# lxa9867/ImageFolder

Measured on NVIDIA H100. Metric: tokenizer_train_images_per_sec_256x256, higher is better.
Workload: dtype bf16

## Files before the change

imagefolder_b200/csrc/attn_kernel.cu:

```cuda
#include "xq_common.cuh"
#include "xq_tc.cuh"

namespace xq {
using namespace xqtc;

constexpr int AT_BM = 128;
constexpr int AT_BN = 128;
constexpr int AT_D = 64;
constexpr int AT_NS = 2;
constexpr int AT_TILE = AT_BM * AT_D * 2;
constexpr int AT_THREADS = 288;

struct AttnFwdSmem {
    static constexpr int Q = 0;
    static constexpr int K = AT_TILE;
    static constexpr int V = AT_TILE * (1 + AT_NS);
    static constexpr int BAR = AT_TILE * (1 + 2 * AT_NS);
    static constexpr int BYTES = BAR + 256;
};

__device__ __forceinline__ void named_bar_sync(int id, int nthreads) { asm volatile("bar.sync %0, %1;" ::"r"(id), "r"(nthreads) : "memory"); }

__global__ void __launch_bounds__(AT_THREADS, 1)
attn_fwd_kernel(const __grid_constant__ CUtensorMap tmQKV, __nv_bfloat16 *__restrict__ out, float *__restrict__ lse2, int N, int H,
// ... 135 lines not shown
attn_fwd_tail_kernel(const __nv_bfloat16 *__restrict__ qkv, __nv_bfloat16 *__restrict__ out, float *__restrict__ lse2, int B, int N,
                     int H, int n0 , float c) {
    const int lane = threadIdx.x & 31;
    const long long w = ((long long)blockIdx.x * blockDim.x + threadIdx.x) >> 5;
    const int nt = N - n0;
    if (w >= (long long)B * H * nt) return;
    const int r = (int)(w % nt);
    const int bh = (int)(w / nt);
    const int b = bh / H, h = bh - b * H;
    const int n = n0 + r;
    const size_t W = (size_t)3 * H * AT_D;
    const __nv_bfloat16 *qp = qkv + ((size_t)b * N + n) * W + h * AT_D;
    float qf[AT_D];
#pragma unroll
    for (int u = 0; u < 8; ++u) {
        const uint4 x = *reinterpret_cast<const uint4 *>(qp + u * 8);
        const __nv_bfloat162 *x2 = reinterpret_cast<const __nv_bfloat162 *>(&x);
#pragma unroll
        for (int e = 0; e < 4; ++e) {
            const float2 f = __bfloat1622float2(x2[e]);
            qf[u * 8 + 2 * e] = f.x * c;
            qf[u * 8 + 2 * e + 1] = f.y * c;
        }
    }
    float m = -CUDART_INF_F, l = 0.f, o[AT_D];
#pragma unroll
    for (int i = 0; i < AT_D; ++i) o[i] = 0.f;
    for (int key = lane; key < N; key += 32) {
        const __nv_bfloat16 *kp = qkv + ((size_t)b * N + key) * W + (H + h) * AT_D;
        const __nv_bfloat16 *vp = kp + (size_t)H * AT_D;
        float s = 0.f;
#pragma unroll
        for (int u = 0; u < 8; ++u) {
            const uint4 x = *reinterpret_cast<const uint4 *>(kp + u * 8);
            const __nv_bfloat162 *x2 = reinterpret_cast<const __nv_bfloat162 *>(&x);
#pragma unroll
            for (int e = 0; e < 4; ++e) {
                const float2 f = __bfloat1622float2(x2[e]);
                s = fmaf(qf[u * 8 + 2 * e], f.x, s);
                s = fmaf(qf[u * 8 + 2 * e + 1], f.y, s);
            }
        }
        const float m_new = fmaxf(m, s);
        const float corr = ex2_approx(m - m_new);
        const float p = ex2_approx(s - m_new);
        l = fmaf(l, corr, p);
        m = m_new;
#pragma unroll
        for (int u = 0; u < 8; ++u) {
            const uint4 x = *reinterpret_cast<const uint4 *>(vp + u * 8);
            const __nv_bfloat162 *x2 = reinterpret_cast<const __nv_bfloat162 *>(&x);
#pragma unroll
            for (int e = 0; e < 4; ++e) {
                const float2 f = __bfloat1622float2(x2[e]);
                o[u * 8 + 2 * e] = fmaf(o[u * 8 + 2 * e], corr, p * f.x);
                o[u * 8 + 2 * e + 1] = fmaf(o[u * 8 + 2 * e + 1], corr, p * f.y);
            }
        }
    }
    float M = m;
#pragma unroll
    for (int off = 16; off > 0; off >>= 1) M = fmaxf(M, __shfl_xor_sync(0xffffffffu, M, off));
    const float f = (m == -CUDART_INF_F) ? 0.f : ex2_approx(m - M);
    l *= f;
#pragma unroll
    for (int off = 16; off > 0; off >>= 1) l += __shfl_xor_sync(0xffffffffu, l, off);
    const float inv = 1.0f / l;
    float mine0 = 0.f, mine1 = 0.f;
#pragma unroll
    for (int i = 0; i < AT_D; ++i) {
        float x = o[i] * f;
#pragma unroll
        for (int off = 16; off > 0; off >>= 1) x += __shfl_xor_sync(0xffffffffu, x, off);
        if (i == 2 * lane) mine0 = x;
        if (i == 2 * lane + 1) mine1 = x;
    }
    __nv_bfloat16 *op = out + ((size_t)b * N + n) * H * AT_D + h * AT_D;
    *reinterpret_cast<uint32_t *>(op + 2 * lane) = pack_bf16(mine0 * inv, mine1 * inv);
    if (lane == 0) lse2[(size_t)bh * N + n] = M + log2f(l);
}

constexpr int AB_THREADS = 288;
constexpr int AB_BQ = 64;
constexpr int AB_QS = 3;
constexpr int AB_QTILE = AB_BQ * AT_D * 2;

struct AttnBwdSmem {
    static constexpr int K = 0;
    static constexpr int V = AT_TILE;
    static constexpr int Q = 2 * AT_TILE;
    static constexpr int DO = Q + AB_QS * AB_QTILE;
    static constexpr int DS = DO + AB_QS * AB_QTILE;
    static constexpr int STAT = DS + 2 * AB_QTILE;
    static constexpr int BAR = STAT + AB_QS * 512;
    static constexpr int BYTES = BAR + 256;
};

__device__ __forceinline__ void bwd_epilogue_frag(const float (&acc)[32], float mul, __nv_bfloat16 *__restrict__ row0,
                                                  size_t row_stride, bool ok0, bool ok1, float *__restrict__ g_bias_cols, int lane) {
    const int cq = 2 * (lane & 3);
#pragma unroll
    for (int jj = 0; jj < AT_D / 8; ++jj) {
        const uint32_t w0 = pack_bf16(acc[4 * jj] * mul, acc[4 * jj + 1] * mul);
        const uint32_t w1 = pack_bf16(acc[4 * jj + 2] * mul, acc[4 * jj + 3] * mul);
        if (ok0) *reinterpret_cast<uint32_t *>(row0 + 8 * jj + cq) = w0;
        if (ok1) *reinterpret_cast<uint32_t *>(row0 + 8 * row_stride + 8 * jj + cq) = w1;
        if (g_bias_cols) {
            float s0 = __uint_as_float(w0 << 16) + __uint_as_float(w1 << 16);
            float s1 = __uint_as_float(w0 & 0xffff0000u) + __uint_as_float(w1 & 0xffff0000u);
#pragma unroll
            for (int o = 4; o < 32; o <<= 1) {
                s0 += __shfl_xor_sync(0xffffffffu, s0, o);
                s1 += __shfl_xor_sync(0xffffffffu, s1, o);
            }
            if (lane < 4) {
                atomicAdd(g_bias_cols + 8 * jj + cq, s0);
                atomicAdd(g_bias_cols + 8 * jj + cq + 1, s1);
            }
        }
    }
}

__global__ void __launch_bounds__(AB_THREADS, 1)
attn_bwd_kernel(const __grid_constant__ CUtensorMap tmQKV, const __grid_constant__ CUtensorMap tmDO, const float *__restrict__ lseP,
                const float *__restrict__ deltaP, float *__restrict__ dq_acc, __nv_bfloat16 *__restrict__ dqkv, float *__restrict__ g_bias,
                int N, int H, int Npad, float c, float scale) {
    extern __shared__ uint8_t smem_raw[];
    uint8_t *base = (uint8_t *)(((uintptr_t)smem_raw + 1023) & ~(uintptr_t)1023);
    uint64_t *bars = (uint64_t *)(base + AttnBwdSmem::BAR);
    uint64_t *kv_full = bars;
    uint64_t *q_full = bars + 1;
    uint64_t *q_empty = bars + 1 + AB_QS;
    float *s_lse = (float *)(base + AttnBwdSmem::STAT);
    float *s_delta = s_lse + AB_QS * AB_BQ;

    const int tid = threadIdx.x, warp = tid >> 5, lane = tid & 31;
    const int bh = blockIdx.y, b = bh / H, h = bh - b * H;
    const int k0 = blockIdx.x * AT_BN;
    const int colQ = h * AT_D, colK = (H + h) * AT_D, colV = (2 * H + h) * AT_D;
    const int nQ = (N + AB_BQ - 1) / AB_BQ;

    if (tid == 0) {
        mbar_init(kv_full, 1);
        for (int i = 0; i < AB_QS; ++i) { mbar_init(&q_full[i], 1); mbar_init(&q_empty[i], 8); }
        mbar_fence_init();
    }
    __syncthreads();

    if (warp == 8) {
        if (elect_one()) {
            tma_prefetch_desc(&tmQKV);
            tma_prefetch_desc(&tmDO);
            mbar_expect_tx(kv_full, 2 * AT_TILE);
            for (int hf = 0; hf < 2; ++hf) {
                tma_load_3d(base + AttnBwdSmem::K + hf * AB_QTILE, &tmQKV, colK, k0 + hf * AB_BQ, b, kv_full);
                tma_load_3d(base + AttnBwdSmem::V + hf * AB_QTILE, &tmQKV, colV, k0 + hf * AB_BQ, b, kv_full);
            }
        }
        __syncwarp();
        for (int i = 0; i < nQ; ++i) {
            const int st = i % AB_QS;
            mbar_wait(&q_empty[st], ((i / AB_QS) & 1) ^ 1);
            if (elect_one()) {
                mbar_expect_tx(&q_full[st], 2 * AB_QTILE + 2 * AB_BQ * 4);
                tma_load_3d(base + AttnBwdSmem::Q + st * AB_QTILE, &tmQKV, colQ, i * AB_BQ, b, &q_full[st]);
                tma_load_3d(base + AttnBwdSmem::DO + st * AB_QTILE, &tmDO, h * AT_D, i * AB_BQ, b, &q_full[st]);
                bulk_g2s(s_lse + st * AB_BQ, lseP + (size_t)bh * Npad + i * AB_BQ, AB_BQ * 4, &q_full[st]);
                bulk_g2s(s_delta + st * AB_BQ, deltaP + (size_t)bh * Npad + i * AB_BQ, AB_BQ * 4, &q_full[st]);
            }
            __syncwarp();
        }
        return;
    }

    const int wg = warp >> 2, wq = warp & 3;
    const int rq = wq * 16 + (lane >> 2), cq = 2 * (lane & 3);
    const int key0 = k0 + wg * 64 + rq;
    const bool kok0 = key0 < N, kok1 = key0 + 8 < N;
    const uint32_t kw = smem_u32(base + AttnBwdSmem::K + wg * AB_QTILE), vw = smem_u32(base + AttnBwdSmem::V + wg * AB_QTILE);
    const uint64_t kd_k = desc_k_sw128(kw), vd_k = desc_k_sw128(vw), kd_mn = desc_mn_sw128(kw, AT_TILE);
    const uint32_t dsw = smem_u32(base + AttnBwdSmem::DS + wg * AB_QTILE);
    const uint64_t dsd = desc_mn_sw128(dsw, AT_TILE);
    float dv[32], dk[32];
#pragma unroll
    for (int i = 0; i < 32; ++i) dv[i] = dk[i] = 0.f;
    mbar_wait(kv_full, 0);
    for (int i = 0; i < nQ; ++i) {
        const int st = i % AB_QS;
        mbar_wait(&q_full[st], (i / AB_QS) & 1);
        const uint32_t qa = smem_u32(base + AttnBwdSmem::Q + st * AB_QTILE), da = smem_u32(base + AttnBwdSmem::DO + st * AB_QTILE);
        float s[32], dp[32];
        wgmma_fence();
#pragma unroll
        for (int k = 0; k < AT_D / 16; ++k) wgmma_m64n64k16_ss<0, 0>(s, desc_adv(kd_k, k * 32), desc_adv(desc_k_sw128(qa), k * 32), (uint32_t)k);
#pragma unroll
        for (int k = 0; k < AT_D / 16; ++k) wgmma_m64n64k16_ss<0, 0>(dp, desc_adv(vd_k, k * 32), desc_adv(desc_k_sw128(da), k * 32), (uint32_t)k);
        wgmma_commit();
        wgmma_wait<0>();
        fence_regs(s);
        fence_regs(dp);
        const float *L = s_lse + st * AB_BQ, *D = s_delta + st * AB_BQ;
        uint32_t pa[4][4], sa[4][4];
#pragma unroll
        for (int jj = 0; jj < AB_BQ / 8; ++jj) {
            const float2 Lq = *reinterpret_cast<const float2 *>(L + 8 * jj + cq);
            const float2 Dq = *reinterpret_cast<const float2 *>(D + 8 * jj + cq);
#pragma unroll
            for (int hh = 0; hh < 2; ++hh) {
                const bool ok = hh ? kok1 : kok0;
                const float p0 = ok ? ex2_approx(fmaf(s[4 * jj + 2 * hh], c, -Lq.x)) : 0.f;
                const float p1 = ok ? ex2_approx(fmaf(s[4 * jj + 2 * hh + 1], c, -Lq.y)) : 0.f;
                const uint32_t pw = pack_bf16(p0, p1);
                const float d0 = __uint_as_float(pw << 16) * (dp[4 * jj + 2 * hh] - Dq.x);
                const float d1 = __uint_as_float(pw & 0xffff0000u) * (dp[4 * jj + 2 * hh + 1] - Dq.y);
                const uint32_t dw = pack_bf16(d0, d1);
                pa[jj >> 1][(jj & 1) * 2 + hh] = pw;
                sa[jj >> 1][(jj & 1) * 2 + hh] = dw;
                asm volatile("st.shared.b32 [%0], %1;" ::"r"(dsw + rowtile_off_bf16(rq + 8 * hh, 8 * jj + cq)), "r"(dw) : "memory");
            }
        }
        fence_async_smem();
        named_bar_sync(1 + wg, 128);
        const uint64_t qd_mn = desc_mn_sw128(qa, AT_TILE), dd_mn = desc_mn_sw128(da, AT_TILE);
        float dq[32];
        wgmma_fence();
#pragma unroll
        for (int k = 0; k < AB_BQ / 16; ++k) {
            wgmma_m64n64k16_rs<1>(dv, pa[k], desc_adv(dd_mn, k * 2048), 1u);
            wgmma_m64n64k16_rs<1>(dk, sa[k], desc_adv(qd_mn, k * 2048), 1u);
        }
#pragma unroll
        for (int k = 0; k < 64 / 16; ++k) wgmma_m64n64k16_ss<1, 1>(dq, desc_adv(dsd, k * 2048), desc_adv(kd_mn, k * 2048), (uint32_t)k);
        wgmma_commit();
        wgmma_wait<0>();
        fence_regs(dv);
        fence_regs(dk);
        fence_regs(dq);
        __syncwarp();
        if (lane == 0) mbar_arrive(&q_empty[st]);
        named_bar_sync(1 + wg, 128);
#pragma unroll
        for (int hh = 0; hh < 2; ++hh) {
            const int q = i * AB_BQ + rq + 8 * hh;
            if (q < N) {
                float *dst = dq_acc + ((size_t)bh * N + q) * AT_D + cq;
#pragma unroll
                for (int jj = 0; jj < AT_D / 8; ++jj)
                    atomicAdd(reinterpret_cast<float2 *>(dst + 8 * jj), make_float2(dq[4 * jj + 2 * hh], dq[4 * jj + 2 * hh + 1]));
            }
        }
    }
    const size_t W = (size_t)3 * H * AT_D;
    __nv_bfloat16 *row = dqkv + ((size_t)b * N + key0) * W;
    bwd_epilogue_frag(dv, 1.0f, row + colV, W, kok0, kok1, g_bias ? g_bias + colV : nullptr, lane);
    bwd_epilogue_frag(dk, scale, row + colK, W, kok0, kok1, g_bias ? g_bias + colK : nullptr, lane);
}


constexpr int AB_KTAIL_MAX = 4;
constexpr int AB_PREP_ROWS = 128;

__device__ __forceinline__ void unpack8(const uint4 &w, float (&f)[8]) {
    const uint32_t x[4] = {w.x, w.y, w.z, w.w};
#pragma unroll
    for (int e = 0; e < 4; ++e) { f[2 * e] = __uint_as_float(x[e] << 16); f[2 * e + 1] = __uint_as_float(x[e] & 0xffff0000u); }
}

template <int NT>
__global__ void __launch_bounds__(256, 2)
attn_bwd_prep_kernel(const __nv_bfloat16 *__restrict__ qkv, const __nv_bfloat16 *__restrict__ out, const __nv_bfloat16 *__restrict__ dout,
                     const float *__restrict__ lse2, float *__restrict__ lseP, float *__restrict__ deltaP, float *__restrict__ dq_acc,
                     float *__restrict__ dsT, __nv_bfloat16 *__restrict__ dqkv, float *__restrict__ g_bias, int N, int H, int Npad,
                     float c, float scale) {
    constexpr int NTA = NT > 0 ? NT : 1;
    __shared__ float red[NT > 0 ? 8 : 1][2][NTA][AT_D];
    __shared__ __align__(16) float skv[2][NTA][AT_D];
    const int bh = blockIdx.y, b = bh / H, h = bh - b * H;
    const int lane = threadIdx.x & 31, sub = threadIdx.x & 7, rloc = threadIdx.x >> 3;
    const int n0 = N - NT;
    const size_t W = (size_t)3 * H * AT_D;
    const __nv_bfloat16 *qb = qkv + (size_t)b * N * W + h * AT_D + sub * 8;
    const size_t ob = (size_t)b * N * H * AT_D + h * AT_D + sub * 8;
    float aK[NTA][8], aV[NTA][8];
    if constexpr (NT > 0) {
        if (threadIdx.x < NT * 16) {
            const int t = threadIdx.x >> 4, isv = (threadIdx.x >> 3) & 1;
            float f[8];
            unpack8(*reinterpret_cast<const uint4 *>(qb + (size_t)(n0 + t) * W + (size_t)(1 + isv) * H * AT_D), f);
#pragma unroll
            for (int e = 0; e < 8; ++e) skv[isv][t][sub * 8 + e] = f[e];
        }
#pragma unroll
        for (int t = 0; t < NT; ++t) {
#pragma unroll
            for (int e = 0; e < 8; ++e) aK[t][e] = aV[t][e] = 0.f;
        }
        __syncthreads();
    }
    constexpr int PASSES = AB_PREP_ROWS / 32;
    extern __shared__ uint4 prep_stage[];
    auto prefetch = [&](int blk, int stg) {
#pragma unroll
        for (int ps = 0; ps < PASSES; ++ps) {
            const int n = blk * AB_PREP_ROWS + ps * 32 + rloc;
            const int nc = n < N ? n : N - 1;
            uint4 *dst = prep_stage + ((size_t)(stg * 3) * PASSES + ps) * 256 + threadIdx.x;
            cp_async16(dst, out + ob + (size_t)nc * H * AT_D);
            cp_async16(dst + PASSES * 256, dout + ob + (size_t)nc * H * AT_D);
            cp_async16(dst + 2 * PASSES * 256, qb + (size_t)nc * W);
        }
        cp_async_commit();
    };
    if constexpr (NT > 0) prefetch(blockIdx.x, 0);
    int stg = 0;
    for (int blk = blockIdx.x; blk * AB_PREP_ROWS < Npad; blk += gridDim.x, stg ^= 1) {
        uint4 ow[PASSES], gw[PASSES], qw[PASSES];
        float lq[PASSES];
#pragma unroll
        for (int ps = 0; ps < PASSES; ++ps) {
            const int n = blk * AB_PREP_ROWS + ps * 32 + rloc;
            const int nc = n < N ? n : N - 1;
            if constexpr (NT == 0) {
                ow[ps] = *reinterpret_cast<const uint4 *>(out + ob + (size_t)nc * H * AT_D);
                gw[ps] = *reinterpret_cast<const uint4 *>(dout + ob + (size_t)nc * H * AT_D);
            }
            lq[ps] = lse2[(size_t)bh * N + nc];
        }
        if constexpr (NT > 0) {
            if ((blk + (int)gridDim.x) * AB_PREP_ROWS < Npad) { prefetch(blk + gridDim.x, stg ^ 1); cp_async_wait<1>(); }
            else cp_async_wait<0>();
        }
#pragma unroll
        for (int ps = 0; ps < PASSES; ++ps) {
            const int n = blk * AB_PREP_ROWS + ps * 32 + rloc;
// ... 130 lines not shown
        }
    }
    if (!g_bias) return;
#pragma unroll
    for (int e = 0; e < 8; ++e) {
        v[e] += __shfl_xor_sync(0xffffffffu, v[e], 8);
        v[e] += __shfl_xor_sync(0xffffffffu, v[e], 16);
    }
    const int warp = threadIdx.x >> 5, lane = threadIdx.x & 31;
    if (lane < 8) {
#pragma unroll
        for (int e = 0; e < 8; ++e) red[warp][lane * 8 + e] = v[e];
    }
    __syncthreads();
    if (threadIdx.x < AT_D) {
        float acc = 0.f;
#pragma unroll
        for (int w8 = 0; w8 < 8; ++w8) acc += red[w8][threadIdx.x];
        atomicAdd(g_bias + hh * AT_D + threadIdx.x, acc);
    }
}

static int attn_bwd_ktail(int N) {
    const int r = N % AT_BN;
    return (N > AT_BN && r != 0 && r <= AB_KTAIL_MAX) ? r : 0;
}

static size_t attn_bwd_ws_layout(int B, int N, int H, size_t *off_lse, size_t *off_delta, size_t *off_dst) {
    const size_t Npad = ((size_t)N + AT_BM - 1) / AT_BM * AT_BM;
    const size_t acc = align_up((size_t)B * H * N * AT_D * sizeof(float), 1024);
    const size_t st = align_up((size_t)B * H * Npad * sizeof(float), 1024);
    const size_t dst = align_up((size_t)B * H * N * attn_bwd_ktail(N) * sizeof(float), 1024);
    if (off_lse) *off_lse = acc;
    if (off_delta) *off_delta = acc + st;
    if (off_dst) *off_dst = acc + 2 * st;
    return acc + 2 * st + dst;
}

}

extern "C" {

size_t xq_vit_attn_bwd_workspace_bytes(int B, int N, int H) {
    if (B <= 0 || N <= 0 || H <= 0) return 0;
    return xq::attn_bwd_ws_layout(B, N, H, nullptr, nullptr, nullptr);
}

int xq_vit_attn_bwd(const void *qkv, const void *out, const void *d_out, const float *lse2, void *dqkv, float *g_bias, int B, int N,
                    int H, int head_dim, float scale, void *workspace, size_t workspace_bytes, void *stream) {
    using namespace xq;
    if (!qkv || !out || !d_out || !lse2 || !dqkv || !workspace || B <= 0 || N <= 0 || H <= 0) return XQ_ERR_ARG;
    if (head_dim != AT_D) return XQ_ERR_UNSUPPORTED;
    if (((uintptr_t)qkv & 15) || ((uintptr_t)out & 15) || ((uintptr_t)d_out & 15) || ((uintptr_t)dqkv & 15) || ((uintptr_t)workspace & 255))
        return XQ_ERR_ARG;
    size_t off_lse, off_delta, off_dst;
    if (workspace_bytes < attn_bwd_ws_layout(B, N, H, &off_lse, &off_delta, &off_dst)) return XQ_ERR_WORKSPACE;
    cudaStream_t st = (cudaStream_t)stream;
    float *acc = (float *)workspace;
    float *lseP = (float *)((char *)workspace + off_lse);
    float *deltaP = (float *)((char *)workspace + off_delta);
    float *dsT = (float *)((char *)workspace + off_dst);
    const uint64_t W = (uint64_t)3 * H * AT_D, Wo = (uint64_t)H * AT_D;
    CUtensorMap tmQKV, tmDO;
    if (!tensor_map_bf16_3d(&tmQKV, qkv, W, N, B, W * 2, (uint64_t)N * W * 2, AB_BQ) ||
        !tensor_map_bf16_3d(&tmDO, d_out, Wo, N, B, Wo * 2, (uint64_t)N * Wo * 2, AB_BQ))
        return XQ_ERR_UNSUPPORTED;
    const int nt = attn_bwd_ktail(N);
    const int nK = nt ? N / AT_BN : (N + AT_BN - 1) / AT_BN;
    const int Npad = (N + AT_BM - 1) / AT_BM * AT_BM;
    if ((long long)B * H > 65535) return XQ_ERR_UNSUPPORTED;
    if (g_bias) XQ_CUDA_TRY(cudaMemsetAsync(g_bias, 0, (size_t)3 * H * AT_D * sizeof(float), st));
    const float c2 = scale * 1.4426950408889634f;
    {
        dim3 grid(nt ? 1u : (unsigned)(Npad / AB_PREP_ROWS), (unsigned)(B * H));
        const size_t ps = nt ? (size_t)2 * 3 * (AB_PREP_ROWS / 32) * 256 * 16 : 0;
        decltype(&attn_bwd_prep_kernel<0>) const preps[] = {attn_bwd_prep_kernel<0>, attn_bwd_prep_kernel<1>, attn_bwd_prep_kernel<2>,
                                                            attn_bwd_prep_kernel<3>, attn_bwd_prep_kernel<4>};
        const auto prep = preps[nt < 4 ? nt : 4];
        if (int rc = smem_optin(prep, ps)) return rc;
        prep<<<grid, 256, ps, st>>>((const __nv_bfloat16 *)qkv, (const __nv_bfloat16 *)out, (const __nv_bfloat16 *)d_out, lse2, lseP,
                                    deltaP, acc, dsT, (__nv_bfloat16 *)dqkv, g_bias, N, H, Npad, c2, scale);
        XQ_LAUNCH_CHECK("attn_bwd_prep_kernel");
    }
    const size_t smem = AttnBwdSmem::BYTES + 1024;
    if (int rc = smem_optin(attn_bwd_kernel, smem)) return rc;
    attn_bwd_kernel<<<dim3((unsigned)nK, (unsigned)(B * H)), AB_THREADS, smem, st>>>(tmQKV, tmDO, lseP, deltaP, acc,
                                                                                     (__nv_bfloat16 *)dqkv, g_bias, N, H, Npad, c2, scale);
    XQ_LAUNCH_CHECK("attn_bwd_kernel");
    {
        dim3 grid((unsigned)((N + AB_CONV_ROWS - 1) / AB_CONV_ROWS), (unsigned)(B * H));
        attn_dq_convert_kernel<<<grid, 256, 0, st>>>(acc, (const __nv_bfloat16 *)qkv, dsT, (__nv_bfloat16 *)dqkv, g_bias, N, H, N - nt, nt, scale);
        XQ_LAUNCH_CHECK("attn_dq_convert_kernel");
    }
    return XQ_OK;
}

int xq_vit_attn_fwd(const void *qkv, void *out, float *lse2, int B, int N, int H, int head_dim, float scale, void *stream) {
    using namespace xq;
    if (!qkv || !out || !lse2 || B <= 0 || N <= 0 || H <= 0) return XQ_ERR_ARG;
    if (head_dim != AT_D) return XQ_ERR_UNSUPPORTED;
    if (((uintptr_t)qkv & 15) || ((uintptr_t)out & 15)) return XQ_ERR_ARG;
    const uint64_t W = (uint64_t)3 * H * AT_D;
    CUtensorMap tmQKV;
    if (!tensor_map_bf16_3d(&tmQKV, qkv, W, N, B, W * 2, (uint64_t)N * W * 2, AT_BM)) return XQ_ERR_UNSUPPORTED;
    const int n_tail = (N % AT_BM != 0 && N % AT_BM <= AT_TAIL_MAX && N > AT_BM) ? N % AT_BM : 0;
    const int nQ = n_tail ? N / AT_BM : (N + AT_BM - 1) / AT_BM;
    const size_t smem = AttnFwdSmem::BYTES + 1024;
    if (int rc = smem_optin(attn_fwd_kernel, smem)) return rc;
    const long long tiles = (long long)B * H * nQ;
    if (tiles > 0x7fffffffLL) return XQ_ERR_ARG;
    const float c = scale * 1.4426950408889634f;
    attn_fwd_kernel<<<(unsigned)tiles, AT_THREADS, smem, (cudaStream_t)stream>>>(tmQKV, (__nv_bfloat16 *)out, lse2, N, H, nQ, c);
    XQ_LAUNCH_CHECK("attn_fwd_kernel");
    if (n_tail) {
        const long long warps = (long long)B * H * n_tail;
        attn_fwd_tail_kernel<<<(unsigned)((warps + 3) / 4), 128, 0, (cudaStream_t)stream>>>(
            (const __nv_bfloat16 *)qkv, (__nv_bfloat16 *)out, lse2, B, N, H, N - n_tail, c);
        XQ_LAUNCH_CHECK("attn_fwd_tail_kernel");
    }
    return XQ_OK;
}

}
```

imagefolder_b200/csrc/xq_tc.cuh:

```cuda
#pragma once
#include <cuda.h>
#include <cuda_bf16.h>
#include <cuda_runtime.h>
#include <stdint.h>

#include <cstring>
#include <mutex>

namespace xqtc {

__device__ __forceinline__ uint32_t smem_u32(const void *p) { return (uint32_t)__cvta_generic_to_shared(p); }

__device__ __forceinline__ void mbar_init(uint64_t *bar, uint32_t count) {
    asm volatile("mbarrier.init.shared::cta.b64 [%0], %1;" ::"r"(smem_u32(bar)), "r"(count));
}
__device__ __forceinline__ void mbar_fence_init() { asm volatile("fence.mbarrier_init.release.cluster;" ::: "memory"); }
__device__ __forceinline__ void mbar_expect_tx(uint64_t *bar, uint32_t bytes) {
    asm volatile("mbarrier.arrive.expect_tx.shared::cta.b64 _, [%0], %1;" ::"r"(smem_u32(bar)), "r"(bytes) : "memory");
}
__device__ __forceinline__ void mbar_arrive(uint64_t *bar) {
    asm volatile("mbarrier.arrive.shared::cta.b64 _, [%0];" ::"r"(smem_u32(bar)) : "memory");
}
__device__ __forceinline__ bool mbar_test(uint64_t *bar, uint32_t parity) {
    uint32_t done;
// ... 24 lines not shown
    asm volatile(
        "{\n\t.reg .pred p;\n\tXQ_MBAR_WAIT:\n\t"
        "mbarrier.try_wait.parity.shared::cta.b64 p, [%0], %1;\n\t"
        "@p bra XQ_MBAR_DONE;\n\tbra XQ_MBAR_WAIT;\n\tXQ_MBAR_DONE:\n\t}" ::"r"(smem_u32(bar)), "r"(parity) : "memory");
}

__device__ __forceinline__ void tma_prefetch_desc(const CUtensorMap *map) {
    asm volatile("prefetch.tensormap [%0];" ::"l"(reinterpret_cast<uint64_t>(map)) : "memory");
}
__device__ __forceinline__ void bulk_g2s(void *dst, const void *src, uint32_t bytes, uint64_t *bar) {
    asm volatile("cp.async.bulk.shared::cluster.global.mbarrier::complete_tx::bytes [%0], [%1], %2, [%3];"
                 ::"r"(smem_u32(dst)), "l"(src), "r"(bytes), "r"(smem_u32(bar))
                 : "memory");
}
__device__ __forceinline__ void tma_load_2d(void *dst, const CUtensorMap *map, int c0, int c1, uint64_t *bar) {
    asm volatile(
        "cp.async.bulk.tensor.2d.shared::cluster.global.mbarrier::complete_tx::bytes [%0], [%1, {%2, %3}], [%4];"
        ::"r"(smem_u32(dst)), "l"(reinterpret_cast<uint64_t>(map)), "r"(c0), "r"(c1), "r"(smem_u32(bar))
        : "memory");
}
__device__ __forceinline__ void tma_load_3d(void *dst, const CUtensorMap *map, int c0, int c1, int c2, uint64_t *bar) {
    asm volatile(
        "cp.async.bulk.tensor.3d.shared::cluster.global.mbarrier::complete_tx::bytes [%0], [%1, {%2, %3, %4}], [%5];"
        ::"r"(smem_u32(dst)), "l"(reinterpret_cast<uint64_t>(map)), "r"(c0), "r"(c1), "r"(c2), "r"(smem_u32(bar))
        : "memory");
}
__device__ __forceinline__ void tma_store_3d(const CUtensorMap *map, const void *src, int c0, int c1, int c2) {
    asm volatile("cp.async.bulk.tensor.3d.global.shared::cta.bulk_group [%0, {%2, %3, %4}], [%1];"
                 ::"l"(reinterpret_cast<uint64_t>(map)), "r"(smem_u32(src)), "r"(c0), "r"(c1), "r"(c2)
                 : "memory");
}
__device__ __forceinline__ void tma_reduce_add_3d(const CUtensorMap *map, const void *src, int c0, int c1, int c2) {
    asm volatile("cp.reduce.async.bulk.tensor.3d.global.shared::cta.add.tile.bulk_group [%0, {%2, %3, %4}], [%1];"
                 ::"l"(reinterpret_cast<uint64_t>(map)), "r"(smem_u32(src)), "r"(c0), "r"(c1), "r"(c2)
                 : "memory");
}
__device__ __forceinline__ void bulk_commit() { asm volatile("cp.async.bulk.commit_group;" ::: "memory"); }
template <int N>
__device__ __forceinline__ void bulk_wait_read() { asm volatile("cp.async.bulk.wait_group.read %0;" ::"n"(N) : "memory"); }
template <int N>
__device__ __forceinline__ void bulk_wait() { asm volatile("cp.async.bulk.wait_group %0;" ::"n"(N) : "memory"); }

__device__ __forceinline__ void fence_async_smem() { asm volatile("fence.proxy.async.shared::cta;" ::: "memory"); }

__device__ __forceinline__ uint64_t desc_k_sw128(uint32_t smem_addr) {
    uint64_t d = 0;
    d |= (uint64_t)((smem_addr & 0x3FFFFu) >> 4);
    d |= (uint64_t)1 << 16;
    d |= (uint64_t)(1024 >> 4) << 32;
    d |= (uint64_t)1 << 62;
    return d;
}
__device__ __forceinline__ uint64_t desc_mn_sw128(uint32_t smem_addr, uint32_t lbo_bytes) {
    uint64_t d = 0;
    d |= (uint64_t)((smem_addr & 0x3FFFFu) >> 4);
    d |= (uint64_t)((lbo_bytes >> 4) & 0x3FFFu) << 16;
    d |= (uint64_t)(1024 >> 4) << 32;
    d |= (uint64_t)1 << 62;
    return d;
}
__device__ __forceinline__ uint64_t desc_adv(uint64_t d, uint32_t bytes) { return d + (uint64_t)(bytes >> 4); }

__device__ __forceinline__ void wgmma_fence() { asm volatile("wgmma.fence.sync.aligned;" ::: "memory"); }
__device__ __forceinline__ void wgmma_commit() { asm volatile("wgmma.commit_group.sync.aligned;" ::: "memory"); }
template <int N>
__device__ __forceinline__ void wgmma_wait() { asm volatile("wgmma.wait_group.sync.aligned %0;" ::"n"(N) : "memory"); }
template <int N>
__device__ __forceinline__ void fence_regs(float (&d)[N]) {
#pragma unroll
    for (int i = 0; i < N; ++i) asm volatile("" : "+f"(d[i])::"memory");
}

template <int TA, int TB>
__device__ __forceinline__ void wgmma_m64n64k16_ss(float (&d)[32], uint64_t da, uint64_t db, uint32_t acc) {
    asm volatile(
        "{\n\t.reg .pred p;\n\tsetp.ne.b32 p, %34, 0;\n\t"
        "wgmma.mma_async.sync.aligned.m64n64k16.f32.bf16.bf16 "
        "{%0, %1, %2, %3, %4, %5, %6, %7, %8, %9, %10, %11, %12, %13, %14, %15, %16, %17, %18, %19, %20, %21, %22, %23, %24, %25, %26, %27, %28, %29, %30, %31}, %32, %33, p, 1, 1, %35, %36;\n\t}"
        : "+f"(d[0]), "+f"(d[1]), "+f"(d[2]), "+f"(d[3]), "+f"(d[4]), "+f"(d[5]), "+f"(d[6]), "+f"(d[7]), "+f"(d[8]), "+f"(d[9]), "+f"(d[10]), "+f"(d[11]), "+f"(d[12]), "+f"(d[13]), "+f"(d[14]), "+f"(d[15]), "+f"(d[16]), "+f"(d[17]), "+f"(d[18]), "+f"(d[19]), "+f"(d[20]), "+f"(d[21]), "+f"(d[22]), "+f"(d[23]), "+f"(d[24]), "+f"(d[25]), "+f"(d[26]), "+f"(d[27]), "+f"(d[28]), "+f"(d[29]), "+f"(d[30]), "+f"(d[31])
        : "l"(da), "l"(db), "r"(acc), "n"(TA), "n"(TB));
}

template <int TA, int TB>
__device__ __forceinline__ void wgmma_m64n128k16_ss(float (&d)[64], uint64_t da, uint64_t db, uint32_t acc) {
    asm volatile(
        "{\n\t.reg .pred p;\n\tsetp.ne.b32 p, %66, 0;\n\t"
        "wgmma.mma_async.sync.aligned.m64n128k16.f32.bf16.bf16 "
        "{%0, %1, %2, %3, %4, %5, %6, %7, %8, %9, %10, %11, %12, %13, %14, %15, %16, %17, %18, %19, %20, %21, %22, %23, %24, %25, %26, %27, %28, %29, %30, %31, %32, %33, %34, %35, %36, %37, %38, %39, %40, %41, %42, %43, %44, %45, %46, %47, %48, %49, %50, %51, %52, %53, %54, %55, %56, %57, %58, %59, %60, %61, %62, %63}, %64, %65, p, 1, 1, %67, %68;\n\t}"
        : "+f"(d[0]), "+f"(d[1]), "+f"(d[2]), "+f"(d[3]), "+f"(d[4]), "+f"(d[5]), "+f"(d[6]), "+f"(d[7]), "+f"(d[8]), "+f"(d[9]), "+f"(d[10]), "+f"(d[11]), "+f"(d[12]), "+f"(d[13]), "+f"(d[14]), "+f"(d[15]), "+f"(d[16]), "+f"(d[17]), "+f"(d[18]), "+f"(d[19]), "+f"(d[20]), "+f"(d[21]), "+f"(d[22]), "+f"(d[23]), "+f"(d[24]), "+f"(d[25]), "+f"(d[26]), "+f"(d[27]), "+f"(d[28]), "+f"(d[29]), "+f"(d[30]), "+f"(d[31]), "+f"(d[32]), "+f"(d[33]), "+f"(d[34]), "+f"(d[35]), "+f"(d[36]), "+f"(d[37]), "+f"(d[38]), "+f"(d[39]), "+f"(d[40]), "+f"(d[41]), "+f"(d[42]), "+f"(d[43]), "+f"(d[44]), "+f"(d[45]), "+f"(d[46]), "+f"(d[47]), "+f"(d[48]), "+f"(d[49]), "+f"(d[50]), "+f"(d[51]), "+f"(d[52]), "+f"(d[53]), "+f"(d[54]), "+f"(d[55]), "+f"(d[56]), "+f"(d[57]), "+f"(d[58]), "+f"(d[59]), "+f"(d[60]), "+f"(d[61]), "+f"(d[62]), "+f"(d[63])
        : "l"(da), "l"(db), "r"(acc), "n"(TA), "n"(TB));
}

template <int TB>
__device__ __forceinline__ void wgmma_m64n64k16_rs(float (&d)[32], const uint32_t (&a)[4], uint64_t db, uint32_t acc) {
    asm volatile(
        "{\n\t.reg .pred p;\n\tsetp.ne.b32 p, %37, 0;\n\t"
        "wgmma.mma_async.sync.aligned.m64n64k16.f32.bf16.bf16 "
        "{%0, %1, %2, %3, %4, %5, %6, %7, %8, %9, %10, %11, %12, %13, %14, %15, %16, %17, %18, %19, %20, %21, %22, %23, %24, %25, %26, %27, %28, %29, %30, %31}, {%32, %33, %34, %35}, %36, p, 1, 1, %38;\n\t}"
        : "+f"(d[0]), "+f"(d[1]), "+f"(d[2]), "+f"(d[3]), "+f"(d[4]), "+f"(d[5]), "+f"(d[6]), "+f"(d[7]), "+f"(d[8]), "+f"(d[9]), "+f"(d[10]), "+f"(d[11]), "+f"(d[12]), "+f"(d[13]), "+f"(d[14]), "+f"(d[15]), "+f"(d[16]), "+f"(d[17]), "+f"(d[18]), "+f"(d[19]), "+f"(d[20]), "+f"(d[21]), "+f"(d[22]), "+f"(d[23]), "+f"(d[24]), "+f"(d[25]), "+f"(d[26]), "+f"(d[27]), "+f"(d[28]), "+f"(d[29]), "+f"(d[30]), "+f"(d[31])
        : "r"(a[0]), "r"(a[1]), "r"(a[2]), "r"(a[3]), "l"(db), "r"(acc), "n"(TB));
}

__device__ __forceinline__ void wgmma_m64n128k8_tf32(float (&d)[64], uint64_t da, uint64_t db, uint32_t acc) {
    asm volatile(
        "{\n\t.reg .pred p;\n\tsetp.ne.b32 p, %66, 0;\n\t"
        "wgmma.mma_async.sync.aligned.m64n128k8.f32.tf32.tf32 "
        "{%0, %1, %2, %3, %4, %5, %6, %7, %8, %9, %10, %11, %12, %13, %14, %15, %16, %17, %18, %19, %20, %21, %22, %23, %24, %25, %26, %27, %28, %29, %30, %31, %32, %33, %34, %35, %36, %37, %38, %39, %40, %41, %42, %43, %44, %45, %46, %47, %48, %49, %50, %51, %52, %53, %54, %55, %56, %57, %58, %59, %60, %61, %62, %63}, %64, %65, p, 1, 1;\n\t}"
        : "+f"(d[0]), "+f"(d[1]), "+f"(d[2]), "+f"(d[3]), "+f"(d[4]), "+f"(d[5]), "+f"(d[6]), "+f"(d[7]), "+f"(d[8]), "+f"(d[9]), "+f"(d[10]), "+f"(d[11]), "+f"(d[12]), "+f"(d[13]), "+f"(d[14]), "+f"(d[15]), "+f"(d[16]), "+f"(d[17]), "+f"(d[18]), "+f"(d[19]), "+f"(d[20]), "+f"(d[21]), "+f"(d[22]), "+f"(d[23]), "+f"(d[24]), "+f"(d[25]), "+f"(d[26]), "+f"(d[27]), "+f"(d[28]), "+f"(d[29]), "+f"(d[30]), "+f"(d[31]), "+f"(d[32]), "+f"(d[33]), "+f"(d[34]), "+f"(d[35]), "+f"(d[36]), "+f"(d[37]), "+f"(d[38]), "+f"(d[39]), "+f"(d[40]), "+f"(d[41]), "+f"(d[42]), "+f"(d[43]), "+f"(d[44]), "+f"(d[45]), "+f"(d[46]), "+f"(d[47]), "+f"(d[48]), "+f"(d[49]), "+f"(d[50]), "+f"(d[51]), "+f"(d[52]), "+f"(d[53]), "+f"(d[54]), "+f"(d[55]), "+f"(d[56]), "+f"(d[57]), "+f"(d[58]), "+f"(d[59]), "+f"(d[60]), "+f"(d[61]), "+f"(d[62]), "+f"(d[63])
        : "l"(da), "l"(db), "r"(acc));
}

__device__ __forceinline__ void sts128(uint32_t saddr, uint4 v) {
    asm volatile("st.shared.v4.b32 [%0], {%1, %2, %3, %4};" ::"r"(saddr), "r"(v.x), "r"(v.y), "r"(v.z), "r"(v.w) : "memory");
}
__device__ __forceinline__ float4 lds128f(uint32_t saddr) {
    float4 v;
    asm volatile("ld.shared.v4.f32 {%0, %1, %2, %3}, [%4];" : "=f"(v.x), "=f"(v.y), "=f"(v.z), "=f"(v.w) : "r"(saddr) : "memory");
    return v;
}

__device__ __forceinline__ bool elect_one() {
    uint32_t pred;
    asm volatile("{\n\t.reg .pred P;\n\telect.sync _|P, 0xffffffff;\n\tselp.b32 %0, 1, 0, P;\n\t}" : "=r"(pred));
    return pred != 0;
}

__host__ __device__ __forceinline__ uint32_t rowtile_off_bf16(int r, int c) {
    return (uint32_t)(r * 128 + ((((c >> 3) ^ (r & 7)) & 7) << 4) + (c & 7) * 2);
}
__host__ __device__ __forceinline__ uint32_t rowtile_unit(int r, int u) { return (uint32_t)(r * 128 + ((u ^ (r & 7)) << 4)); }

__device__ __forceinline__ uint32_t pack_bf16(float lo, float hi) {
    uint32_t r;
    asm("cvt.rn.bf16x2.f32 %0, %1, %2;" : "=r"(r) : "f"(hi), "f"(lo));
    return r;
}
__device__ __forceinline__ float ex2_approx(float x) {
    float y;
    asm("ex2.approx.ftz.f32 %0, %1;" : "=f"(y) : "f"(x));
    return y;
}

constexpr int TMAP_CACHE = 128;

inline bool tensor_map(CUtensorMap *out, const void *base, CUtensorMapDataType dtype, int rank, const cuuint64_t *dims,
                       const cuuint64_t *strides, const cuuint32_t *box, CUtensorMapSwizzle swizzle) {
    typedef CUresult (*Encode)(CUtensorMap *, CUtensorMapDataType, cuuint32_t, void *, const cuuint64_t *, const cuuint64_t *,
                               const cuuint32_t *, const cuuint32_t *, CUtensorMapInterleave, CUtensorMapSwizzle,
                               CUtensorMapL2promotion, CUtensorMapFloatOOBfill);
    struct Entry { uint64_t key[12]; CUtensorMap map; };
    static std::mutex mu;
    static Entry cache[TMAP_CACHE];
    static int n_cached = 0, next = 0;
    static Encode encode = nullptr;
    if (rank < 1 || rank > 3) return false;
    uint64_t key[12] = {(uint64_t)(uintptr_t)base, (uint64_t)dtype, (uint64_t)rank, (uint64_t)swizzle};
    for (int i = 0; i < rank; ++i) { key[4 + i] = dims[i]; key[7 + i] = box[i]; }
    for (int i = 0; i + 1 < rank; ++i) key[10 + i] = strides[i];
    std::lock_guard<std::mutex> g(mu);
    for (int i = 0; i < n_cached; ++i)
        if (memcmp(cache[i].key, key, sizeof(key)) == 0) { *out = cache[i].map; return true; }
    if (!encode) {
        void *p = nullptr;
        cudaDriverEntryPointQueryResult q;
        if (cudaGetDriverEntryPoint("cuTensorMapEncodeTiled", &p, cudaEnableDefault, &q) != cudaSuccess ||
            q != cudaDriverEntryPointSuccess)
            return false;
        encode = (Encode)p;
    }
    const cuuint32_t estr[3] = {1u, 1u, 1u};
    CUtensorMap m;
    if (encode(&m, dtype, (cuuint32_t)rank, const_cast<void *>(base), dims, strides, box, estr, CU_TENSOR_MAP_INTERLEAVE_NONE,
               swizzle, CU_TENSOR_MAP_L2_PROMOTION_L2_256B, CU_TENSOR_MAP_FLOAT_OOB_FILL_NONE) != CUDA_SUCCESS)
        return false;
    memcpy(cache[next].key, key, sizeof(key));
    cache[next].map = m;
    next = (next + 1) % TMAP_CACHE;
    if (n_cached < TMAP_CACHE) ++n_cached;
    *out = m;
    return true;
}

inline bool tensor_map_bf16_3d(CUtensorMap *out, const void *base, uint64_t inner, uint64_t rows, uint64_t batch,
                               uint64_t row_stride_bytes, uint64_t batch_stride_bytes, uint32_t box_rows) {
    const cuuint64_t dims[3] = {inner, rows, batch}, strides[2] = {row_stride_bytes, batch_stride_bytes};
    const cuuint32_t box[3] = {64u, box_rows, 1u};
    return tensor_map(out, base, CU_TENSOR_MAP_DATA_TYPE_BFLOAT16, 3, dims, strides, box, CU_TENSOR_MAP_SWIZZLE_128B);
}

}
```

Measured before the change: 644.4.

## Accumulate dQ via TMA reduce-add from shared tiles with cross-warpgroup split and narrow tail

Replaces per-thread global float2 atomicAdds of dQ in the attention backward with a double-buffered shared dQ tile that a single thread reduces into global memory using TMA reduce-add. The dQ GEMM is split across both warpgroups over all 128 keys (each computes half the head dim), which requires a 256-thread barrier and double-buffered dS written with stmatrix. A templated narrow-tail path uses n16 MMAs for a final partial Q block. It also adds optional clock instrumentation. In exchange it uses more shared memory and adds cross-warpgroup synchronization each iteration.

```diff
diff --git a/imagefolder_b200/csrc/attn_kernel.cu b/imagefolder_b200/csrc/attn_kernel.cu
--- a/imagefolder_b200/csrc/attn_kernel.cu
+++ b/imagefolder_b200/csrc/attn_kernel.cu
@@ -241,8 +241,10 @@
 
 constexpr int AB_THREADS = 288;
 constexpr int AB_BQ = 64;
+constexpr int AB_TQ = 16;
 constexpr int AB_QS = 3;
 constexpr int AB_QTILE = AB_BQ * AT_D * 2;
+constexpr int AB_DQTILE = AB_BQ * AT_D * 4;
 
 struct AttnBwdSmem {
     static constexpr int K = 0;
@@ -250,10 +252,35 @@
     static constexpr int Q = 2 * AT_TILE;
     static constexpr int DO = Q + AB_QS * AB_QTILE;
     static constexpr int DS = DO + AB_QS * AB_QTILE;
-    static constexpr int STAT = DS + 2 * AB_QTILE;
+    static constexpr int DQ = DS + 4 * AB_QTILE;
+    static constexpr int STAT = DQ + 2 * AB_DQTILE;
     static constexpr int BAR = STAT + AB_QS * 512;
     static constexpr int BYTES = BAR + 256;
 };
+
+enum { AT_CLK_QWAIT, AT_CLK_MMA1, AT_CLK_DS, AT_CLK_BAR1, AT_CLK_MMA2, AT_CLK_DQ, AT_CLK_BLOCKS, AT_CLK_SLOTS };
+#ifdef XQ_AT_CLOCKS
+__device__ unsigned long long at_clocks[AT_CLK_SLOTS];
+struct AtClock {
+    uint32_t t, acc[AT_CLK_SLOTS] = {};
+    __device__ void start() { t = (uint32_t)clock(); }
+    __device__ void lap(int slot) { const uint32_t n = (uint32_t)clock(); acc[slot] += n - t; t = n; }
+    __device__ void count(int slot) { ++acc[slot]; }
+    __device__ void flush(bool me) {
+        if (!me) return;
+#pragma unroll
+        for (int i = 0; i < AT_CLK_SLOTS; ++i)
+            if (acc[i]) atomicAdd(&at_clocks[i], (unsigned long long)acc[i]);
+    }
+};
+#else
+struct AtClock {
+    __device__ void start() {}
+    __device__ void lap(int) {}
+    __device__ void count(int) {}
+    __device__ void flush(bool) {}
+};
+#endif
 
 __device__ __forceinline__ void bwd_epilogue_frag(const float (&acc)[32], float mul, __nv_bfloat16 *__restrict__ row0,
                                                   size_t row_stride, bool ok0, bool ok1, float *__restrict__ g_bias_cols, int lane) {
@@ -280,9 +307,121 @@
     }
 }
 
+template <int NDQ>
+__device__ __forceinline__ void wgmma_dq(float (&d)[NDQ / 2], uint64_t da, uint64_t db, uint32_t acc) {
+    if constexpr (NDQ == 32) wgmma_m64n32k16_ss<1, 0>(d, da, db, acc);
+    else wgmma_m64n8k16_ss<1, 0>(d, da, db, acc);
+}
+
+__device__ __forceinline__ void attn_bwd_dq_reduce(const CUtensorMap *tmDQ, uint8_t *base, int i, int bh) {
+    uint8_t *tile = base + AttnBwdSmem::DQ + (i & 1) * AB_DQTILE;
+    tma_reduce_add_3d(tmDQ, tile, 0, i * AB_BQ, bh);
+    tma_reduce_add_3d(tmDQ, tile + AB_DQTILE / 2, 32, i * AB_BQ, bh);
+    bulk_commit();
+}
+
+template <int NB>
+__device__ __forceinline__ void attn_bwd_block(int i, float (&dv)[32], float (&dk)[32], AtClock &clk, uint8_t *base, uint64_t *q_full,
+                                               uint64_t *q_empty, const float *s_lse, const float *s_delta, const CUtensorMap *tmDQ,
+                                               int bh, int wg, int lane, int rq, int cq, bool kok0, bool kok1, float c) {
+    constexpr int NDQ = NB / 2;
+    const int st = i % AB_QS, par = i & 1;
+    const bool issuer = threadIdx.x == 0;
+    clk.start();
+    mbar_wait(&q_full[st], (i / AB_QS) & 1);
+    clk.lap(AT_CLK_QWAIT);
+    const uint32_t qa = smem_u32(base + AttnBwdSmem::Q + st * AB_QTILE), da = smem_u32(base + AttnBwdSmem::DO + st * AB_QTILE);
+    const uint64_t kd_k = desc_k_sw128(smem_u32(base + AttnBwdSmem::K + wg * AB_QTILE));
+    const uint64_t vd_k = desc_k_sw128(smem_u32(base + AttnBwdSmem::V + wg * AB_QTILE));
+    float s[NB / 2], dp[NB / 2];
+    wgmma_fence();
+#pragma unroll
+    for (int k = 0; k < AT_D / 16; ++k) {
+        if constexpr (NB == AB_BQ) wgmma_m64n64k16_ss<0, 0>(s, desc_adv(kd_k, k * 32), desc_adv(desc_k_sw128(qa), k * 32), (uint32_t)k);
+        else wgmma_m64n16k16_ss<0, 0>(s, desc_adv(kd_k, k * 32), desc_adv(desc_k_sw128(qa), k * 32), (uint32_t)k);
+    }
+#pragma unroll
+    for (int k = 0; k < AT_D / 16; ++k) {
+        if constexpr (NB == AB_BQ) wgmma_m64n64k16_ss<0, 0>(dp, desc_adv(vd_k, k * 32), desc_adv(desc_k_sw128(da), k * 32), (uint32_t)k);
+        else wgmma_m64n16k16_ss<0, 0>(dp, desc_adv(vd_k, k * 32), desc_adv(desc_k_sw128(da), k * 32), (uint32_t)k);
+    }
+    wgmma_commit();
+    wgmma_wait<0>();
+    fence_regs(s);
+    fence_regs(dp);
+    clk.lap(AT_CLK_MMA1);
+    const float *L = s_lse + st * AB_BQ, *D = s_delta + st * AB_BQ;
+    const uint32_t dsw = smem_u32(base + AttnBwdSmem::DS + (2 * par + wg) * AB_QTILE);
+    uint32_t pa[NB / 16][4], sa[NB / 16][4];
+#pragma unroll
+    for (int jj = 0; jj < NB / 8; ++jj) {
+        const float2 Lq = *reinterpret_cast<const float2 *>(L + 8 * jj + cq);
+        const float2 Dq = *reinterpret_cast<const float2 *>(D + 8 * jj + cq);
+#pragma unroll
+        for (int hh = 0; hh < 2; ++hh) {
+            const bool ok = hh ? kok1 : kok0;
+            const float p0 = ok ? ex2_approx(fmaf(s[4 * jj + 2 * hh], c, -Lq.x)) : 0.f;
+            const float p1 = ok ? ex2_approx(fmaf(s[4 * jj + 2 * hh + 1], c, -Lq.y)) : 0.f;
+            const uint32_t pw = pack_bf16(p0, p1);
+            const float d0 = __uint_as_float(pw << 16) * (dp[4 * jj + 2 * hh] - Dq.x);
+            const float d1 = __uint_as_float(pw & 0xffff0000u) * (dp[4 * jj + 2 * hh + 1] - Dq.y);
+            const uint32_t dw = pack_bf16(d0, d1);
+            pa[jj >> 1][(jj & 1) * 2 + hh] = pw;
+            sa[jj >> 1][(jj & 1) * 2 + hh] = dw;
+        }
+        if (jj & 1)
+            stmatrix_x4_trans(dsw + (jj >> 1) * 2048 + rowtile_off_bf16(8 * (lane >> 4) + (lane & 7), (rq & 48) + 8 * ((lane >> 3) & 1)),
+                              sa[jj >> 1]);
+    }
+    fence_async_smem();
+    clk.lap(AT_CLK_DS);
+    if (issuer) bulk_wait_read<0>();
+    named_bar_sync(1, 256);
+    if (issuer && i > 0) attn_bwd_dq_reduce(tmDQ, base, i - 1, bh);
+    clk.lap(AT_CLK_BAR1);
+    const uint64_t qd_mn = desc_mn_sw128(qa, AT_TILE), dd_mn = desc_mn_sw128(da, AT_TILE);
+    const uint64_t kd_mn = desc_mn_sw128(smem_u32(base + AttnBwdSmem::K), AT_TILE);
+    const uint32_t dsq = smem_u32(base + AttnBwdSmem::DS + 2 * par * AB_QTILE) + wg * NDQ * 128;
+    float dq[NDQ / 2];
+    wgmma_fence();
+#pragma unroll
+    for (int k = 0; k < NB / 16; ++k) {
+        wgmma_m64n64k16_rs<1>(dv, pa[k], desc_adv(dd_mn, k * 2048), 1u);
+        wgmma_m64n64k16_rs<1>(dk, sa[k], desc_adv(qd_mn, k * 2048), 1u);
+    }
+#pragma unroll
+    for (int k = 0; k < AT_BN / 16; ++k)
+        wgmma_dq<NDQ>(dq, desc_adv(kd_mn, k * 2048), desc_adv(desc_k_sw128(dsq + (k >> 2) * AB_QTILE), (k & 3) * 32), (uint32_t)k);
+    wgmma_commit();
+    wgmma_wait<0>();
+    fence_regs(dv);
+    fence_regs(dk);
+    fence_regs(dq);
+    clk.lap(AT_CLK_MMA2);
+    __syncwarp();
+    if (lane == 0) mbar_arrive(&q_empty[st]);
+    uint8_t *tile = base + AttnBwdSmem::DQ + par * AB_DQTILE;
+    const uint32_t ts = smem_u32(tile) + (rq >> 5) * (AB_DQTILE / 2) + wg * NDQ * 128;
+    uint32_t to[4];
+#pragma unroll
+    for (int e = 0; e < 4; ++e) {
+        const int q = cq + (e & 1), d = (rq & 31) + 8 * (e >> 1);
+        to[e] = q * 128 + (((d >> 2) ^ q) << 4) + (d & 3) * 4;
+    }
+#pragma unroll
+    for (int j = 0; j < NDQ / 8; ++j) {
+#pragma unroll
+        for (int e = 0; e < 4; ++e) asm volatile("st.shared.f32 [%0], %1;" ::"r"(ts + j * 1024 + to[e]), "f"(dq[4 * j + e]) : "memory");
+    }
+    fence_async_smem();
+    clk.lap(AT_CLK_DQ);
+    clk.count(AT_CLK_BLOCKS);
+}
+
+template <bool NARROW_TAIL>
 __global__ void __launch_bounds__(AB_THREADS, 1)
-attn_bwd_kernel(const __grid_constant__ CUtensorMap tmQKV, const __grid_constant__ CUtensorMap tmDO, const float *__restrict__ lseP,
-                const float *__restrict__ deltaP, float *__restrict__ dq_acc, __nv_bfloat16 *__restrict__ dqkv, float *__restrict__ g_bias,
+attn_bwd_kernel(const __grid_constant__ CUtensorMap tmQKV, const __grid_constant__ CUtensorMap tmDO, const __grid_constant__ CUtensorMap tmDQ,
+                const float *__restrict__ lseP, const float *__restrict__ deltaP, __nv_bfloat16 *__restrict__ dqkv, float *__restrict__ g_bias,
                 int N, int H, int Npad, float c, float scale) {
     extern __shared__ uint8_t smem_raw[];
     uint8_t *base = (uint8_t *)(((uintptr_t)smem_raw + 1023) & ~(uintptr_t)1023);
@@ -310,6 +449,7 @@
         if (elect_one()) {
             tma_prefetch_desc(&tmQKV);
             tma_prefetch_desc(&tmDO);
+            tma_prefetch_desc(&tmDQ);
             mbar_expect_tx(kv_full, 2 * AT_TILE);
             for (int hf = 0; hf < 2; ++hf) {
                 tma_load_3d(base + AttnBwdSmem::K + hf * AB_QTILE, &tmQKV, colK, k0 + hf * AB_BQ, b, kv_full);
@@ -336,79 +476,22 @@
     const int rq = wq * 16 + (lane >> 2), cq = 2 * (lane & 3);
     const int key0 = k0 + wg * 64 + rq;
     const bool kok0 = key0 < N, kok1 = key0 + 8 < N;
-    const uint32_t kw = smem_u32(base + AttnBwdSmem::K + wg * AB_QTILE), vw = smem_u32(base + AttnBwdSmem::V + wg * AB_QTILE);
-    const uint64_t kd_k = desc_k_sw128(kw), vd_k = desc_k_sw128(vw), kd_mn = desc_mn_sw128(kw, AT_TILE);
-    const uint32_t dsw = smem_u32(base + AttnBwdSmem::DS + wg * AB_QTILE);
-    const uint64_t dsd = desc_mn_sw128(dsw, AT_TILE);
     float dv[32], dk[32];
 #pragma unroll
     for (int i = 0; i < 32; ++i) dv[i] = dk[i] = 0.f;
+    AtClock clk;
     mbar_wait(kv_full, 0);
-    for (int i = 0; i < nQ; ++i) {
-        const int st = i % AB_QS;
-        mbar_wait(&q_full[st], (i / AB_QS) & 1);
-        const uint32_t qa = smem_u32(base + AttnBwdSmem::Q + st * AB_QTILE), da = smem_u32(base + AttnBwdSmem::DO + st * AB_QTILE);
-        float s[32], dp[32];
-        wgmma_fence();
-#pragma unroll
-        for (int k = 0; k < AT_D / 16; ++k) wgmma_m64n64k16_ss<0, 0>(s, desc_adv(kd_k, k * 32), desc_adv(desc_k_sw128(qa), k * 32), (uint32_t)k);
-#pragma unroll
-        for (int k = 0; k < AT_D / 16; ++k) wgmma_m64n64k16_ss<0, 0>(dp, desc_adv(vd_k, k * 32), desc_adv(desc_k_sw128(da), k * 32), (uint32_t)k);
-        wgmma_commit();
-        wgmma_wait<0>();
-        fence_regs(s);
-        fence_regs(dp);
-        const float *L = s_lse + st * AB_BQ, *D = s_delta + st * AB_BQ;
-        uint32_t pa[4][4], sa[4][4];
-#pragma unroll
-        for (int jj = 0; jj < AB_BQ / 8; ++jj) {
-            const float2 Lq = *reinterpret_cast<const float2 *>(L + 8 * jj + cq);
-            const float2 Dq = *reinterpret_cast<const float2 *>(D + 8 * jj + cq);
-#pragma unroll
-            for (int hh = 0; hh < 2; ++hh) {
-                const bool ok = hh ? kok1 : kok0;
-                const float p0 = ok ? ex2_approx(fmaf(s[4 * jj + 2 * hh], c, -Lq.x)) : 0.f;
-                const float p1 = ok ? ex2_approx(fmaf(s[4 * jj + 2 * hh + 1], c, -Lq.y)) : 0.f;
-                const uint32_t pw = pack_bf16(p0, p1);
-                const float d0 = __uint_as_float(pw << 16) * (dp[4 * jj + 2 * hh] - Dq.x);
-                const float d1 = __uint_as_float(pw & 0xffff0000u) * (dp[4 * jj + 2 * hh + 1] - Dq.y);
-                const uint32_t dw = pack_bf16(d0, d1);
-                pa[jj >> 1][(jj & 1) * 2 + hh] = pw;
-                sa[jj >> 1][(jj & 1) * 2 + hh] = dw;
-                asm volatile("st.shared.b32 [%0], %1;" ::"r"(dsw + rowtile_off_bf16(rq + 8 * hh, 8 * jj + cq)), "r"(dw) : "memory");
-            }
-        }
-        fence_async_smem();
-        named_bar_sync(1 + wg, 128);
-        const uint64_t qd_mn = desc_mn_sw128(qa, AT_TILE), dd_mn = desc_mn_sw128(da, AT_TILE);
-        float dq[32];
-        wgmma_fence();
-#pragma unroll
-        for (int k = 0; k < AB_BQ / 16; ++k) {
-            wgmma_m64n64k16_rs<1>(dv, pa[k], desc_adv(dd_mn, k * 2048), 1u);
-            wgmma_m64n64k16_rs<1>(dk, sa[k], desc_adv(qd_mn, k * 2048), 1u);
-        }
-#pragma unroll
-        for (int k = 0; k < 64 / 16; ++k) wgmma_m64n64k16_ss<1, 1>(dq, desc_adv(dsd, k * 2048), desc_adv(kd_mn, k * 2048), (uint32_t)k);
-        wgmma_commit();
-        wgmma_wait<0>();
-        fence_regs(dv);
-        fence_regs(dk);
-        fence_regs(dq);
-        __syncwarp();
-        if (lane == 0) mbar_arrive(&q_empty[st]);
-        named_bar_sync(1 + wg, 128);
-#pragma unroll
-        for (int hh = 0; hh < 2; ++hh) {
-            const int q = i * AB_BQ + rq + 8 * hh;
-            if (q < N) {
-                float *dst = dq_acc + ((size_t)bh * N + q) * AT_D + cq;
-#pragma unroll
-                for (int jj = 0; jj < AT_D / 8; ++jj)
-                    atomicAdd(reinterpret_cast<float2 *>(dst + 8 * jj), make_float2(dq[4 * jj + 2 * hh], dq[4 * jj + 2 * hh + 1]));
-            }
-        }
-    }
+    const int nFull = NARROW_TAIL ? nQ - 1 : nQ;
+    for (int i = 0; i < nFull; ++i)
+        attn_bwd_block<AB_BQ>(i, dv, dk, clk, base, q_full, q_empty, s_lse, s_delta, &tmDQ, bh, wg, lane, rq, cq, kok0, kok1, c);
+    if constexpr (NARROW_TAIL)
+        attn_bwd_block<AB_TQ>(nQ - 1, dv, dk, clk, base, q_full, q_empty, s_lse, s_delta, &tmDQ, bh, wg, lane, rq, cq, kok0, kok1, c);
+    named_bar_sync(1, 256);
+    if (tid == 0) {
+        attn_bwd_dq_reduce(&tmDQ, base, nQ - 1, bh);
+        bulk_wait<0>();
+    }
+    clk.flush((tid & 127) == 0);
     const size_t W = (size_t)3 * H * AT_D;
     __nv_bfloat16 *row = dqkv + ((size_t)b * N + key0) * W;
     bwd_epilogue_frag(dv, 1.0f, row + colV, W, kok0, kok1, g_bias ? g_bias + colV : nullptr, lane);
@@ -705,11 +788,20 @@
                                     deltaP, acc, dsT, (__nv_bfloat16 *)dqkv, g_bias, N, H, Npad, c2, scale);
         XQ_LAUNCH_CHECK("attn_bwd_prep_kernel");
     }
-    const size_t smem = AttnBwdSmem::BYTES + 1024;
-    if (int rc = smem_optin(attn_bwd_kernel, smem)) return rc;
-    attn_bwd_kernel<<<dim3((unsigned)nK, (unsigned)(B * H)), AB_THREADS, smem, st>>>(tmQKV, tmDO, lseP, deltaP, acc,
-                                                                                     (__nv_bfloat16 *)dqkv, g_bias, N, H, Npad, c2, scale);
-    XQ_LAUNCH_CHECK("attn_bwd_kernel");
+    {
+        CUtensorMap tmDQ;
+        const cuuint64_t dims[3] = {AT_D, (cuuint64_t)N, (cuuint64_t)B * H}, strides[2] = {AT_D * 4, (cuuint64_t)N * AT_D * 4};
+        const cuuint32_t box[3] = {32, AB_BQ, 1};
+        if (!tensor_map(&tmDQ, acc, CU_TENSOR_MAP_DATA_TYPE_FLOAT32, 3, dims, strides, box, CU_TENSOR_MAP_SWIZZLE_128B))
+            return XQ_ERR_UNSUPPORTED;
+        const int tq = N % AB_BQ;
+        const auto kern = (tq != 0 && tq <= AB_TQ) ? attn_bwd_kernel<true> : attn_bwd_kernel<false>;
+        const size_t smem = AttnBwdSmem::BYTES + 1024;
+        if (int rc = smem_optin(kern, smem)) return rc;
+        kern<<<dim3((unsigned)nK, (unsigned)(B * H)), AB_THREADS, smem, st>>>(tmQKV, tmDO, tmDQ, lseP, deltaP, (__nv_bfloat16 *)dqkv,
+                                                                           g_bias, N, H, Npad, c2, scale);
+        XQ_LAUNCH_CHECK("attn_bwd_kernel");
+    }
     {
         dim3 grid((unsigned)((N + AB_CONV_ROWS - 1) / AB_CONV_ROWS), (unsigned)(B * H));
         attn_dq_convert_kernel<<<grid, 256, 0, st>>>(acc, (const __nv_bfloat16 *)qkv, dsT, (__nv_bfloat16 *)dqkv, g_bias, N, H, N - nt, nt, scale);
@@ -717,6 +809,15 @@
     }
     return XQ_OK;
 }
+
+#ifdef XQ_AT_CLOCKS
+int xq_at_clocks_read(unsigned long long *out) {
+    XQ_CUDA_TRY(cudaMemcpyFromSymbol(out, xq::at_clocks, sizeof(xq::at_clocks)));
+    unsigned long long zero[xq::AT_CLK_SLOTS] = {};
+    XQ_CUDA_TRY(cudaMemcpyToSymbol(xq::at_clocks, zero, sizeof(zero)));
+    return XQ_OK;
+}
+#endif
 
 int xq_vit_attn_fwd(const void *qkv, void *out, float *lse2, int B, int N, int H, int head_dim, float scale, void *stream) {
     using namespace xq;
diff --git a/imagefolder_b200/csrc/xq_tc.cuh b/imagefolder_b200/csrc/xq_tc.cuh
--- a/imagefolder_b200/csrc/xq_tc.cuh
+++ b/imagefolder_b200/csrc/xq_tc.cuh
@@ -130,6 +130,36 @@
 }
 
 template <int TA, int TB>
+__device__ __forceinline__ void wgmma_m64n8k16_ss(float (&d)[4], uint64_t da, uint64_t db, uint32_t acc) {
+    asm volatile(
+        "{\n\t.reg .pred p;\n\tsetp.ne.b32 p, %6, 0;\n\t"
+        "wgmma.mma_async.sync.aligned.m64n8k16.f32.bf16.bf16 "
+        "{%0, %1, %2, %3}, %4, %5, p, 1, 1, %7, %8;\n\t}"
+        : "+f"(d[0]), "+f"(d[1]), "+f"(d[2]), "+f"(d[3])
+        : "l"(da), "l"(db), "r"(acc), "n"(TA), "n"(TB));
+}
+
+template <int TA, int TB>
+__device__ __forceinline__ void wgmma_m64n32k16_ss(float (&d)[16], uint64_t da, uint64_t db, uint32_t acc) {
+    asm volatile(
+        "{\n\t.reg .pred p;\n\tsetp.ne.b32 p, %18, 0;\n\t"
+        "wgmma.mma_async.sync.aligned.m64n32k16.f32.bf16.bf16 "
+        "{%0, %1, %2, %3, %4, %5, %6, %7, %8, %9, %10, %11, %12, %13, %14, %15}, %16, %17, p, 1, 1, %19, %20;\n\t}"
+        : "+f"(d[0]), "+f"(d[1]), "+f"(d[2]), "+f"(d[3]), "+f"(d[4]), "+f"(d[5]), "+f"(d[6]), "+f"(d[7]), "+f"(d[8]), "+f"(d[9]), "+f"(d[10]), "+f"(d[11]), "+f"(d[12]), "+f"(d[13]), "+f"(d[14]), "+f"(d[15])
+        : "l"(da), "l"(db), "r"(acc), "n"(TA), "n"(TB));
+}
+
+template <int TA, int TB>
+__device__ __forceinline__ void wgmma_m64n16k16_ss(float (&d)[8], uint64_t da, uint64_t db, uint32_t acc) {
+    asm volatile(
+        "{\n\t.reg .pred p;\n\tsetp.ne.b32 p, %10, 0;\n\t"
+        "wgmma.mma_async.sync.aligned.m64n16k16.f32.bf16.bf16 "
+        "{%0, %1, %2, %3, %4, %5, %6, %7}, %8, %9, p, 1, 1, %11, %12;\n\t}"
+        : "+f"(d[0]), "+f"(d[1]), "+f"(d[2]), "+f"(d[3]), "+f"(d[4]), "+f"(d[5]), "+f"(d[6]), "+f"(d[7])
+        : "l"(da), "l"(db), "r"(acc), "n"(TA), "n"(TB));
+}
+
+template <int TA, int TB>
 __device__ __forceinline__ void wgmma_m64n128k16_ss(float (&d)[64], uint64_t da, uint64_t db, uint32_t acc) {
     asm volatile(
         "{\n\t.reg .pred p;\n\tsetp.ne.b32 p, %66, 0;\n\t"
@@ -160,6 +190,11 @@
 
 __device__ __forceinline__ void sts128(uint32_t saddr, uint4 v) {
     asm volatile("st.shared.v4.b32 [%0], {%1, %2, %3, %4};" ::"r"(saddr), "r"(v.x), "r"(v.y), "r"(v.z), "r"(v.w) : "memory");
+}
+__device__ __forceinline__ void stmatrix_x4_trans(uint32_t saddr, const uint32_t (&r)[4]) {
+    asm volatile("stmatrix.sync.aligned.m8n8.x4.trans.shared.b16 [%0], {%1, %2, %3, %4};" ::"r"(saddr), "r"(r[0]), "r"(r[1]), "r"(r[2]),
+                 "r"(r[3])
+                 : "memory");
 }
 __device__ __forceinline__ float4 lds128f(uint32_t saddr) {
     float4 v;
```

Result: faster. 672.6, median of 6 (+4.4%).
